# tgcsaba/GPSig

Hardware: AMD Instinct MI355X
Metric: sequence-pairs/sec for SignatureKernel.K (N,L,d,sig_level); fp64 rel-err vs ref (higher is better)
Workload: dtype f64; 1 GPU; BASELINE.json configs[1]: full N x N Gram, SignatureLinear, N=4096, L=64, d=8, num_levels=5, order=1, normalization=on, fp64, white-noise inputs

## Files before the change

gpsig_amd/csrc/ctx.hpp:

```cpp
#pragma once
#include <atomic>

#include <hip/hip_runtime.h>

#include <cstdarg>
#include <cstdio>
#include <cstdlib>
#include <cstring>
#include <string>
#include <thread>
#include <vector>

#include "../../include/gpsig_hip.h"
#include "seq_args.hpp"

struct DevBuf {
    void* p = nullptr;
    size_t cap = 0;
};

struct UploadCache {
    uint64_t hash = 0;
    void* base = nullptr;
    std::vector<size_t> offsets;
};

enum BufId {
    B_IN0, B_IN1, B_IN2,
    B_OUT0, B_OUT1, B_OUT2,
    B_REC0, B_REC1,
    B_DLEV0, B_DLEV1,
    B_FAC0, B_FAC1,
    B_TASKS, B_W, B_XT, B_ZT, B_ZS, B_ZL, B_ZN, B_TMP0, B_TMP1,
    B_LS, B_LR0, B_LR1, B_LR2, B_LR3, B_LR4, B_LR5, B_LR6, B_LR7, B_LR8,
    B_GR0, B_GR1, B_GR2, B_GR3, B_GR4, B_GR5, B_GR6, B_GR7,
    B_GR7B, B_TW0, B_TW1, B_TW2,
    B_SF0, B_SF1, B_SF2, B_SF3, B_SF4, B_SF5,
    B_SPEC,
    B_SPECD, B_LRDK,
    B_SPECW,
    B_LRF32,
    B_TQ,
    B_STASH,
    B_WD0, B_WD1, B_WD2, B_WD3, B_WD4, B_WD5, B_WD6, B_WD7, B_WD8, B_WD9, B_WD10, B_WD11, B_WD12, B_WD13, B_WD14, B_WD15,
    B_WS0, B_WS1, B_WS2, B_WS3,
    B_RG0, B_RG1, B_RG2, B_RG3, B_RG4,
    B_COUNT
};

inline thread_local std::string g_create_error;

struct TaskCache {
    int64_t key[10] = {0};
    int ntasks = 0;
    bool valid = false;
    bool match(const int64_t (&k)[10]) const {
        if (!valid) return false;
        for (int i = 0; i < 10; ++i) if (key[i] != k[i]) return false;
        return true;
    }
    void set(const int64_t (&k)[10], int n) { for (int i = 0; i < 10; ++i) key[i] = k[i]; ntasks = n; valid = true; }
};

struct TaskSlot {
    TaskCache tc;
    DevBuf buf;
    uint64_t stamp = 0;
    int64_t aux = 0;
};
constexpr size_t TASK_SLOTS = 16;

inline int64_t next_stash_generation() {
    static std::atomic<int64_t> counter{0};
    return ++counter;
}

struct gpsig_ctx {
    int device = 0;
    int num_cus = 256;
    hipStream_t stream = nullptr;
    int ptr_mode = GPSIG_PTR_HOST;
    int shard_i = 0, shard_n = 1;
    int use_glds = 1;
    int allow_exact = 1;
    int keep_reset = 1;
    int f32_pack = 2, f32_waves = 0;
    int allow_pk2 = 1;
    int max_run = 0;
    int tens_lanes = -1;
    int grad_scratch_mb = 4096;
    int matern_fast = 1;
    int grad_fused_piece = 0;
    int grad_stash_mb = 4096;
    bool stash_want = false;
    int64_t stash_desc[8] = {0, 0, 0, 0, 0, 0, 0, 0};
    int64_t stash_gen = 0;
    int grad_impl = 0;
    void* blas_handle = nullptr;
    int tvs_tile = -1;
// ... 400 lines not shown
```

gpsig_amd/csrc/launchers.hpp:

```cpp
#pragma once
#include <hip/hip_runtime.h>

#include <cstddef>
#include <cstdint>
#include <string>

struct gpsig_ctx;
struct gpsig_params;

namespace gpsig {
struct ScaleParams;
struct SeqGramArgs;
struct TvsArgs;
struct TvsLaneTArgs;
struct TvsTileArgs;
struct TvsGradTileArgs;
struct SigFeatArgs;
struct SigGramArgs;
struct SigReduceArgs;
struct SigFeatGradArgs;
struct WaveGradArgs;
struct Wave2Args;
struct WaveHoArgs;
struct FusedGradArgs;
// ... 41 lines not shown
GPSIG_SEQ_UNITS(GPSIG_SEQ_UNIT_DECL)
GPSIG_SEQ_HO_UNITS(GPSIG_SEQ_HO_UNIT_DECL)
#undef GPSIG_SEQ_UNIT_DECL
#undef GPSIG_SEQ_HO_UNIT_DECL
SeqLaunchFn seq_lookup_ptdrbf_stash(int G, int C, int D, int MMAX);
SeqLaunchFn seq_lookup_ptdmatern_stash(int kind, int G, int C, int D, int MMAX);
SeqLaunchFn seq_lookup_ho_ptdrbf_exact(int G, int C, int D, int M, int order);
SeqLaunchFn seq_lookup_ho_ptdrbf_exact_o4(int G, int C, int D, int M, int order);
SeqLaunchFn seq_lookup_ho_ptdm12_exact(int kind, int G, int C, int D, int M, int order);
SeqLaunchFn seq_lookup_ho_ptdm32_exact(int kind, int G, int C, int D, int M, int order);
SeqLaunchFn seq_lookup_ho_ptdm52_exact(int kind, int G, int C, int D, int M, int order);
bool seq_pk2_select(int rows, int d, int M, int* G, int* C, int* D);
SeqLaunchFn seq_pk2_lookup(int G, int C, int D, int M, int mode, int pack, int waves);

TvsLaunchFn tvs_lookup(int M, int TT, bool incr, bool f32);
#define GPSIG_TENS_DECL(tag) TvsLaunchFn tvs_lookup_##tag##_lo(int, int, bool); TvsLaunchFn tvs_lookup_##tag##_m6(int, int, bool); \
                             TvsLaunchFn tvs_lookup_##tag##_m7(int, int, bool); TvsLaunchFn tvs_lookup_##tag##_m8(int, int, bool);
GPSIG_TENS_DECL(f64) GPSIG_TENS_DECL(f32)
#undef GPSIG_TENS_DECL
bool tvs_lanet_plan(int M, int d, bool incr, TvsLaneTLaunchFn* fns, int* ngroups);
int tvs_tile_width(int d);
int tvs_tile_waves(int M, int D, int E, int kind);
TvsTileLaunchFn tvs_tile_lookup(int M, int NW, int D, bool incr, int kind);
TvsTileLaunchFn tvs_tile_lookup_m2(int, int, bool, int);
TvsTileLaunchFn tvs_tile_lookup_m3(int, int, bool, int);
TvsTileLaunchFn tvs_tile_lookup_m4(int, int, bool, int);
TvsTileLaunchFn tvs_tile_lookup_m5(int, int, bool, int);
TvsTileLaunchFn tvs_tile_lookup_m6(int, int, bool, int);
TvsTileLaunchFn tvs_tile_lookup_ho(int M, int NW, int D, bool incr);
TvsGradTileLaunchFn tvs_grad_tile_lookup_m1(int, int, bool);
TvsGradTileLaunchFn tvs_grad_tile_lookup_m2(int, int, bool);
TvsGradTileLaunchFn tvs_grad_tile_lookup_m3(int, int, bool);
TvsGradTileLaunchFn tvs_grad_tile_lookup_m4(int, int, bool);
TvsGradTileLaunchFn tvs_grad_tile_lookup_m5(int, int, bool);
TvsGradTileLaunchFn tvs_grad_tile_lookup_m6(int, int, bool);
TvsGradTileLaunchFn tvs_grad_tile_lookup_ho(int M, int D, bool paired, int kind);
bool tvs_grad_tile_ho_available(const gpsig_ctx* c, const gpsig_params* p, int d, int L, int increments);
int tvs_grad_tile_device(gpsig_ctx* c, const gpsig_params* p, int d, const double* Z, const double* X, const double* G, int64_t Tn, int64_t N,
                         int L, int increments, const double* fac, const double* aux, double* gZ, double* gX, double* gfac, double* gb, size_t budget, bool* done);

SigFeatLaunchFn sig_feat_lookup(int d, int M);
SigFeatLaunchFn sig_feat_pick_a(int d, int M);
SigFeatLaunchFn sig_feat_pick_b(int d, int M);
SigFeatLaunchFn sig_feat_pick_c(int d, int M);
SigFeatLaunchFn sig_feat_pick_d(int d, int M);
SigFeatLaunchFn sig_feat_pick_e(int d, int M);
SigFeatLaunchFn sig_feat_pick_f(int d, int M);
SigFeatGradLaunchFn sig_feat_grad_pick_a(int d, int M);
SigFeatGradLaunchFn sig_feat_grad_pick_b(int d, int M);
SigFeatGradLaunchFn sig_feat_grad_pick_c(int d, int M);
SigFeatGradLaunchFn sig_feat_grad_pick_d(int d, int M);
SigFeatGradLaunchFn sig_feat_grad_pick_e(int d, int M);
SigFeatGradLaunchFn sig_feat_grad_pick_f(int d, int M);
hipError_t sig_gram_launch(const SigGramArgs& G, int ntiles, hipStream_t stream, int dma, int* used_dma);
hipError_t sig_reduce_launch(const SigReduceArgs& R, hipStream_t stream);
hipError_t sig_convert_launch(const void* in, void* out, int64_t n, bool widen, hipStream_t stream);
struct SigShape { int d, M; bool cosine; int64_t F, ld; SigFeatLaunchFn ffn; };
bool sig_shape(const gpsig_params* p, int d, SigShape* s);
constexpr size_t SIG_FEAT_LDS_MAX = 150 * 1024, SIG_FEAT_GRAD_LDS_MAX = 158 * 1024;
bool sig_shape_fits(const SigShape& s, const gpsig_params* p, int L);
int sig_launch_features(gpsig_ctx* c, const SigShape& s, const gpsig_params* p, const ScaleParams& P, int order, const double* X, int64_t N, int L,
                        const double* w, int normalize, double jitter, int norm_squared, int natural_order, double* Phi, double* dlev);
int sig_features_K(gpsig_ctx* c, const gpsig_params* p, bool raw, const void* X, const void* X2, int64_t N1, int64_t N2, int L1, int L2, int return_levels,
                   void* out, bool timed, int x_squared, int64_t row_begin, int64_t row_end, int compact, bool* done, bool row_block_call = false);
bool tvs_features_plan(gpsig_ctx* c, const gpsig_params* p, bool f64, int64_t Tn, int64_t N, int L);
int tens_vs_seq_features_device(gpsig_ctx* c, const gpsig_params* p, bool f64, const void* ZT, const void* ZS, const void* X, int64_t Tn, int64_t N, int L,
                                int increments, const double* w, void* out, bool* done);
int sig_features_grad(gpsig_ctx* c, const gpsig_params* p, int d, const double* X, const double* Y, int64_t N1, int64_t N2, int L1, int L2, bool diag,
                      bool sym, const double* G, double* gX, double* gY, bool* done);

WaveLaunchFn wave_lookup_inc(int G, int C, int DP, int LQ);
WaveLaunchFn wave_lookup_ptd(int G, int C, int DP, int LQ);
WaveLaunchFn wave_lookup_ptn(int G, int C, int DP, int LQ);
Wave2LaunchFn wave2_lookup_inc(int G, int C, int DP, int LQ);
Wave2LaunchFn lam_undo_lookup_ptd_rbf(int G, int C, int DP, int LQ);
Wave2LaunchFn lam_undo_lookup_ptd_gen(int G, int C, int DP, int LQ);
Wave2LaunchFn lam_undo_lookup_ptn_rbf(int G, int C, int DP, int LQ);
Wave2LaunchFn lam_undo_lookup_ptn_gen(int G, int C, int DP, int LQ);
WaveHoLaunchFn wave_ho_lookup(int G, int C, int order, int M);
WaveHoLaunchFn wave_o1_lookup(int G, int C, int M);
WaveHoLaunchFn wave_ho_undo_lookup_g16(int C, int order, int M);
WaveHoLaunchFn wave_ho_undo_lookup_g32(int C, int order, int M);
WaveHoLaunchFn wave_ho_undo_lookup_g64(int C, int order, int M);
WaveHoLaunchFn wave_ho_levels_lookup_g16(int C, int order, int M);
WaveHoLaunchFn wave_ho_levels_lookup_g32(int C, int order, int M);
WaveHoLaunchFn wave_ho_levels_lookup_g64(int C, int order, int M);
FusedGradLaunchFn fused_grad_stash_lookup(int kind, int DP, int LQ);
FusedGradLaunchFn fused_grad_lookup_diff_g16(int kind, int DP, int LQ);
FusedGradLaunchFn fused_grad_lookup_diff_g32(int kind, int DP, int LQ);
FusedGradLaunchFn fused_grad_lookup_diff_g64(int kind, int DP, int LQ);
FusedGradLaunchFn fused_grad_lookup_nodiff_g16(int kind, int DP, int LQ);
FusedGradLaunchFn fused_grad_lookup_nodiff_g32(int kind, int DP, int LQ);
FusedGradLaunchFn fused_grad_lookup_nodiff_g64(int kind, int DP, int LQ);
struct HoSweeps { WaveHoLaunchFn fn; int G, C; size_t lds, slot; };
bool ho_sweeps_plan(const gpsig_ctx* c, const gpsig_params* p, int R1, int R2, HoSweeps* hs);
bool o1_sweeps_plan(const gpsig_ctx* c, const gpsig_params* p, int R1, int R2, HoSweeps* hs);
bool ho_levels_plan(const gpsig_ctx* c, const gpsig_params* p, int R1, int R2, HoSweeps* hs);
int ho_sweeps_launch(gpsig_ctx* c, const HoSweeps& hs, int M, int R1, int R2, const double* dM, double* lam, const double* G, int64_t gm, int64_t gi,
                     int64_t gj, int64_t N2, bool diag, int64_t pair0, int64_t npairs);
int ho_levels_launch(gpsig_ctx* c, const HoSweeps& hs, int M, int R1, int R2, const double* dM, double* out, int64_t gm, int64_t gi, int64_t gj, int64_t N2,
                     bool diag, int64_t pair0, int64_t npairs);

bool wide_tvs_available(const gpsig_ctx* c, const gpsig_params* p, int d, int64_t Tn, int64_t N, int L);
int wide_tvs_forward(gpsig_ctx* c, const gpsig_params* p, const ScaleParams& sz, int d, const double* Z, const double* Xs, int64_t Tn, int64_t N, int L,
                     int increments, const double* fx, const double* w, int sum_levels, double* out, double* aux);
int wide_tvs_backward(gpsig_ctx* c, const gpsig_params* p, int d, const double* Z, const double* X, const double* G, int64_t Tn, int64_t N, int L,
                      int increments, const double* fac, const double* aux, double* gZ, double* gX, double* gfac, double* g_base);
// ... 44 lines not shown
```

gpsig_amd/csrc/sig_feat_api.hip:

```cpp
#include "api_common.hpp"
#include "launchers.hpp"
#include "sig_feat_kernel.hpp"

namespace {

static __global__ void tens_level_features_kernel(const double* __restrict__ ZT, const double* __restrict__ ZS, int lt, int E, int d, int64_t Tn,
                                                  int M, int unit, int64_t ld, double* __restrict__ Zf) {
    const int64_t total = Tn * ld;
    for (int64_t e = blockIdx.x * int64_t(blockDim.x) + threadIdx.x; e < total; e += int64_t(gridDim.x) * blockDim.x) {
        const int64_t t = e / ld;
        int k = int(e - t * ld), m = 1, w = d, off = 0;
        while (m <= M && k >= off + w) { off += w; ++m; w *= d; }
        double v;
        if (m > M) {
            v = k == off ? 1.0 : 0.0;
        } else {
            int idx = k - off;
            const int c0 = m * (m - 1) / 2;
            v = 1.0;
            for (int j = m - 1; j >= 0; --j) {
                const int f = idx % d;
                idx /= d;
                const int c = c0 + j;
                double z = ZT[((t * d + f) * lt + c) * E + (E - 1)];
// ... 104 lines not shown
uint64_t sig_keep_key(const gpsig_params* p, bool raw, int x_squared, int64_t N1, int L1, int64_t ld) {
    const int32_t head[8] = {p->base_kernel, p->dtype, p->num_features, p->num_levels, p->order, p->difference, p->normalization, p->num_lags};
    const int64_t tail[4] = {N1, L1, (raw ? 1 : 0) + (x_squared ? 2 : 0), ld};
    uint64_t key = fnv1a(FNV1A_BASIS, head, sizeof(head));
    key = fnv1a(fnv1a(key, &p->sigma, sizeof(double)), &p->jitter, sizeof(double));
    key = fnv1a(key, p->variances, sizeof(double) * (p->num_levels + 1));
    if (p->lengthscales) key = fnv1a(key, p->lengthscales, sizeof(double) * p->num_features);
    if (p->num_lags > 0) key = fnv1a(fnv1a(key, p->lags, sizeof(double) * p->num_lags), p->gamma, sizeof(double) * (p->num_lags + 1));
    return fnv1a(key, tail, sizeof(tail));
}

int sig_gram_stage_f32(gpsig_ctx* c, const gpsig_params* p, const SigGramPlan& g, int L1, int L2, int return_levels, const void** X, const void** X2,
                       void** out) {
    void *x64, *y64 = nullptr, *o64;
    const int64_t per1 = int64_t(L1) * p->num_features, per2 = int64_t(L2) * p->num_features;
    CHK(ensure(c, B_SF3, sizeof(double) * size_t(g.N1 * per1) + 64, &x64));
    HIPCHK(c, sig_convert_launch(*X, x64, g.N1 * per1, true, c->stream));
    if (!g.sym) {
        CHK(ensure(c, B_SF4, sizeof(double) * size_t(g.N2 * per2) + 64, &y64));
        HIPCHK(c, sig_convert_launch(*X2, y64, g.N2 * per2, true, c->stream));
    }
    CHK(ensure(c, B_SF5, sizeof(double) * size_t(return_levels ? p->num_levels + 1 : 1) * size_t(g.N1) * size_t(g.sym ? g.N1 : g.N2) + 64, &o64));
    *X = x64; *X2 = g.sym ? nullptr : y64; *out = o64;
    return GPSIG_OK;
}

int sig_gram_levels(gpsig_ctx* c, const gpsig_params* p, const SigShape& s, const SigGramPlan& g, bool raw, int return_levels, int normalize,
                    const void* phi1, const void* phi2, void* part, void* out, bool timed, int compact) {
    const int M = s.M, d = s.d;
    const int64_t F = s.F, ld = s.ld, N1 = g.N1, NA = g.NA, NB = g.NB, H = g.H, row_begin = g.row_begin, Ncols = g.sym ? N1 : g.N2;
    const bool rows = g.rows;
    const int nlev = return_levels ? M + 1 : 1;
    for (int lv = 0; lv < nlev; ++lv) {
        int kb = 0, ke = int(F) + 1;
        double dval = 0.0;
        if (return_levels) {
            if (lv == 0) { kb = int(F); ke = int(F) + 1; }
            else { kb = sig_feature_count(d, lv - 1); ke = sig_feature_count(d, lv); }
            dval = raw ? 0.0 : p->sigma * p->variances[lv];
        } else {
            for (int m = 0; m <= M; ++m) dval += p->sigma * p->variances[m];
        }
        SigGramArgs G;
        memset(&G, 0, sizeof(G));
        G.A = static_cast<const double*>(phi1) + (rows ? row_begin * ld : 0);
        G.B = static_cast<const double*>(g.sym ? phi1 : phi2);
        G.NA = NA; G.NB = NB; G.lda = ld; G.ldb = ld;
        G.b_off = rows ? ((row_begin - H) % N1 + N1) % N1 : 0; G.b_mod = g.sym ? N1 : g.N2;
        G.k_begin = kb; G.k_end = ke;
        G.band = (rows && NA + H <= N1) ? H : 0;
        const int nslab = (ke - kb + SG_BK - 1) / SG_BK;
        const int ns = sig_piece_bounds(nslab, g.nsplit, return_levels ? 1 : g.graded, G.bound);
        G.nsplit = ns; G.symmetric = g.symtiles ? 1 : 0; G.ntj = g.ntj; G.part = static_cast<double*>(part);
        hipEvent_t e0 = nullptr, e1 = nullptr;
        bool on = false;
        if (timed) CHK(timing_begin(c, &e0, &e1, &on));
        int used_dma = 0;
        HIPCHK(c, sig_gram_launch(G, g.ntiles, c->stream, (c->sig_gemm_dma && !return_levels) ? 1 : 0, &used_dma));
        if (on) {
            HIPCHK(c, hipEventRecord(e1, c->stream));
            c->t_launches += 1;
            c->t_pairs += NA * NB;
            c->t_kernel = used_dma ? "sig_gram_dma_kernel" : "sig_gram_kernel";
            const double tiles_done = double(g.ntiles) - ((used_dma && g.symtiles) ? double(g.nti) * 28.0 / 64.0 : 0.0);
            c->t_flops += 2.0 * tiles_done * SG_BM * SG_BN * double(nslab) * SG_BK;
        }
        SigReduceArgs R;
        memset(&R, 0, sizeof(R));
        R.part = static_cast<const double*>(part); R.nsplit = ns; R.NA = NA; R.NB = NB;
        R.out = static_cast<double*>(out) + (return_levels ? int64_t(lv) * N1 * Ncols : 0);
        R.so_i = Ncols; R.so_j = 1;
        R.mode = rows ? 2 : (g.symtiles ? 1 : 0);
        R.diag_set = (g.sym && normalize) ? 1 : 0; R.diag_value = dval;
        R.N = N1; R.r0 = row_begin; R.c0 = G.b_off; R.compact = compact;
        HIPCHK(c, sig_reduce_launch(R, c->stream));
    }
    return GPSIG_OK;
}

}

int sig_features_K(gpsig_ctx* c, const gpsig_params* p, bool raw, const void* X, const void* X2, int64_t N1, int64_t N2, int L1, int L2,
                   int return_levels, void* out, bool timed, int x_squared, int64_t row_begin, int64_t row_end, int compact, bool* done,
                   bool row_block_call) {
    *done = false;
    const bool sym = X2 == nullptr, f32 = p->dtype == GPSIG_F32;
    const bool rows = row_end > 0 || row_block_call;
    SigShape s;
    if (!sig_gram_route(c, p, raw, sym, rows, N1, N2, L1, L2, x_squared, &s)) return GPSIG_OK;
    SigGramPlan g = sig_gram_geometry(sym, rows, N1, N2, row_begin, row_end);
    const int nslab_all = int((s.ld + SG_BK - 1) / SG_BK);
    sig_piece_counts(N1, N2, sym, nslab_all, c->sig_graded != 0, &g.nsplit, &g.graded);
    const size_t part_one = sizeof(double) * size_t(g.NA) * g.NB;
    while (g.nsplit > 1 && part_one * size_t(g.nsplit - 1 + g.graded) > (size_t(40) << 30)) { --g.nsplit; g.graded = 1; }
    const int npieces = g.nsplit - 1 + g.graded;
    const size_t feat_bytes = sizeof(double) * size_t(s.ld) * (size_t(N1) + (sym ? 0 : size_t(N2)));
    if (feat_bytes + part_one * size_t(npieces) > (size_t(96) << 30)) return GPSIG_OK;
    const SigBuf bufs[3] = {{B_SF0, sizeof(double) * size_t(s.ld) * N1 + 64}, {B_SF1, sym ? 0 : sizeof(double) * size_t(s.ld) * N2 + 64},
                            {B_SF2, part_one * size_t(npieces) + 64}};
    if (!sig_gram_headroom(c, bufs, rows)) return GPSIG_OK;
    if (rows && g.NA <= 0) { *done = true; return GPSIG_OK; }
    const double* w = nullptr;
    if (!raw) CHK(upload_weights(c, p, &w));
    ScaleParams sp;
    CHK(scale_params(c, p, !raw, &sp));
    void* dev[3] = {nullptr, nullptr, nullptr};
    for (int i = 0; i < 3; ++i)
        if (bufs[i].bytes) CHK(ensure(c, bufs[i].id, bufs[i].bytes, &dev[i]));
    void* const phi1 = dev[0];
    void* out32 = nullptr;
    const void* const X_given = X;
    if (f32) {
        out32 = out;
        CHK(sig_gram_stage_f32(c, p, g, L1, L2, return_levels, &X, &X2, &out));
    }
    const int normalize = (!raw && p->normalization) ? 1 : 0;
    const uint64_t key = sig_keep_key(p, raw, x_squared, N1, L1, s.ld);
    const bool reuse = c->sf_keep && c->sf_valid && c->sf_X == X_given && c->sf_phi == phi1 && c->sf_key == key;
    if (N1 > 0 && !reuse)
        CHK(sig_launch_features(c, s, p, sp, p->order, static_cast<const double*>(X), N1, L1, w, normalize, p->jitter, x_squared ? 1 : 0, 0,
                                static_cast<double*>(phi1), nullptr));
    c->sf_valid = c->sf_keep != 0 && N1 > 0;
    c->sf_X = X_given; c->sf_phi = phi1; c->sf_key = key;
    if (!sym && N2 > 0)
        CHK(sig_launch_features(c, s, p, sp, p->order, static_cast<const double*>(X2), N2, L2, w, normalize, p->jitter, 0, 0,
                                static_cast<double*>(dev[1]), nullptr));
    if (g.NA <= 0 || g.NB <= 0) { *done = true; return GPSIG_OK; }
    CHK(sig_gram_levels(c, p, s, g, raw, return_levels, normalize, phi1, dev[1], dev[2], out, timed, compact));
// ... 66 lines not shown
```

gpsig_amd/csrc/sig_feat_inst.hip:

```cpp
#include "launchers.hpp"
#include "sig_feat_kernel.hpp"

namespace gpsig {
SigFeatLaunchFn sig_feat_lookup(int d, int M) {
    if (d < 1 || d > 32) return nullptr;
    return d <= 4 ? sig_feat_pick_a(d, M) : d <= 8 ? sig_feat_pick_b(d, M) : d <= 12 ? sig_feat_pick_c(d, M) : d <= 16 ? sig_feat_pick_d(d, M)
         : d <= 24 ? sig_feat_pick_e(d, M) : sig_feat_pick_f(d, M);
}

hipError_t sig_gram_launch(const SigGramArgs& G, int ntiles, hipStream_t stream, int dma, int* used_dma) {
    if (used_dma) *used_dma = 0;
    const bool aligned = (G.lda % 2) == 0 && (G.ldb % 2) == 0 && (reinterpret_cast<uintptr_t>(G.A) % 16) == 0 &&
                         (reinterpret_cast<uintptr_t>(G.B) % 16) == 0;
    const int ke_pad = (G.k_end + SG_BK - 1) / SG_BK * SG_BK;
    if (dma && aligned && G.k_begin % SG_BK == 0 && ke_pad <= G.lda && ke_pad <= G.ldb) {
        hipLaunchKernelGGL(sig_gram_dma_kernel, dim3(unsigned(ntiles) * unsigned(G.nsplit)), dim3(256), 0, stream, G);
        if (used_dma) *used_dma = 1;
        return hipGetLastError();
    }
    const bool vec = (G.k_begin % 2) == 0 && (G.lda % 2) == 0 && (G.ldb % 2) == 0 && (reinterpret_cast<uintptr_t>(G.A) % 16) == 0 &&
                     (reinterpret_cast<uintptr_t>(G.B) % 16) == 0;
    if (vec) hipLaunchKernelGGL(sig_gram_kernel<true>, dim3(unsigned(ntiles) * unsigned(G.nsplit)), dim3(256), 0, stream, G);
    else hipLaunchKernelGGL(sig_gram_kernel<false>, dim3(unsigned(ntiles) * unsigned(G.nsplit)), dim3(256), 0, stream, G);
    return hipGetLastError();
}
hipError_t sig_convert_launch(const void* in, void* out, int64_t n, bool widen, hipStream_t stream) {
    if (n <= 0) return hipSuccess;
    int64_t g = (n + 255) / 256;
    if (g > 16384) g = 16384;
    if (widen) hipLaunchKernelGGL(sig_widen_kernel, dim3(unsigned(g)), dim3(256), 0, stream, static_cast<const float*>(in), static_cast<double*>(out), n);
    else hipLaunchKernelGGL(sig_narrow_kernel, dim3(unsigned(g)), dim3(256), 0, stream, static_cast<const double*>(in), static_cast<float*>(out), n);
    return hipGetLastError();
}
hipError_t sig_reduce_launch(const SigReduceArgs& R, hipStream_t stream) {
    if (R.mode == 1) {
        const int nt = int((R.NA + SG_BM - 1) / SG_BM);
        hipLaunchKernelGGL(sig_gram_reduce_sym_kernel, dim3((SG_BM / 32) * (SG_BM / 32), unsigned(nt * (nt + 1) / 2)), dim3(32, 8), 0, stream, R, nt);
        return hipGetLastError();
    }
    int64_t g = (R.NA * R.NB + 255) / 256;
    if (g > 65536) g = 65536;
    if (g < 1) g = 1;
    hipLaunchKernelGGL(sig_gram_reduce_kernel, dim3(unsigned(g)), dim3(256), 0, stream, R);
    return hipGetLastError();
}
}
```

gpsig_amd/csrc/sig_feat_kernel.hpp:

```cpp
#pragma once

#include <hip/hip_runtime.h>
#include <stdint.h>

#include <type_traits>

#include "aux_kernels.hpp"
#include "sig_pieces.hpp"

namespace gpsig {

constexpr int sig_ipow(int d, int m) {
    long long v = 1;
    for (int i = 0; i < m; ++i) { v *= d; if (v > (1ll << 30)) return 1 << 30; }
    return int(v);
}
constexpr int sig_lower_total(int d, int M) { int s = 0; for (int m = 1; m < M; ++m) s += sig_ipow(d, m); return s; }
constexpr int sig_feature_count(int d, int M) { int s = 0; for (int m = 1; m <= M; ++m) s += sig_ipow(d, m); return s; }
constexpr int SIG_MAX_TOP = 32768;
constexpr int sig_threads(int d, int M) {
    int t = 64;
    while (t < 512 && t * 64 < sig_ipow(d, M)) t *= 2;
    return t;
}
// ... 348 lines not shown
                double2* o2 = reinterpret_cast<double2*>(out + off);
#pragma unroll
                for (int q = 0; q < D; ++q)
#pragma unroll
                    for (int f = 0; f < D; f += 2) o2[(q * (D / 2) + f / 2) * T + tid] = double2{sc * top[q][f], sc * top[q][f + 1]};
            } else {
#pragma unroll
                for (int q = 0; q < D; ++q)
#pragma unroll
                    for (int f = 0; f < D; ++f) out[off + (q * D + f) * T + tid] = sc * top[q][f];
            }
            off += sig_ipow(D, M);
        }
        for (int64_t e = off + tid; e < A.ld; e += T) out[e] = e == off ? scale_of(0) : 0.0;
        if (A.dlev && tid <= M) A.dlev[n * (M + 1) + tid] = tid == 0 ? 1.0 : norms[tid];
    }
}

inline size_t sig_features_lds_bytes(int d, int M, int L) {
    (void)M;
    return sizeof(double) * ((size_t(L) + (d <= 64 ? 64 / d : 1)) * d + 64 + 64 + size_t(L) * d + size_t(L));
}

#ifdef GPSIG_KERNEL_DEFS
__global__ void sig_widen_kernel(const float* __restrict__ in, double* __restrict__ out, int64_t n) {
    for (int64_t i = blockIdx.x * int64_t(blockDim.x) + threadIdx.x; i < n; i += int64_t(gridDim.x) * blockDim.x) out[i] = double(in[i]);
}
#else
__global__ void sig_widen_kernel(const float* __restrict__ in, double* __restrict__ out, int64_t n);
#endif
#ifdef GPSIG_KERNEL_DEFS
__global__ void sig_narrow_kernel(const double* __restrict__ in, float* __restrict__ out, int64_t n) {
    for (int64_t i = blockIdx.x * int64_t(blockDim.x) + threadIdx.x; i < n; i += int64_t(gridDim.x) * blockDim.x) out[i] = float(in[i]);
}
#else
__global__ void sig_narrow_kernel(const double* __restrict__ in, float* __restrict__ out, int64_t n);
#endif

typedef double sig_f64x4 __attribute__((ext_vector_type(4)));
constexpr int SG_BM = 128, SG_BN = 128, SG_BK = 16, SG_LDK = SG_BK + 1;
constexpr int SG_MAX_PIECES = 144;

struct SigGramArgs {
    const double* A; const double* B;
    int64_t NA, NB, lda, ldb;
    int64_t b_off, b_mod;
    int k_begin, k_end;
    int nsplit;
    int bound[SG_MAX_PIECES + 1];
    int symmetric;
    int ntj;
    double* part;
    int64_t band;
};

__device__ inline void sig_tile_of(const SigGramArgs& G, int& split_out, int& bi, int& bj) {
    const int ntiles = gridDim.x / G.nsplit;
    const int split = blockIdx.x / ntiles;
    int tile;
    {
        const int j = blockIdx.x - split * ntiles, off = (split * ntiles) & 7, x = (off + j) & 7;
        int start = 0;
        for (int xp = 0; xp < x; ++xp) {
            const int j0 = (xp - off + 8) & 7;
            start += j0 < ntiles ? (ntiles - 1 - j0) / 8 + 1 : 0;
        }
        tile = start + ((j - ((x - off + 8) & 7)) >> 3);
    }
    {
        constexpr int SB = 8;
        if (G.symmetric) {
            const int d = int(int64_t(tile) * G.ntj / ntiles);
            if (int(int64_t(tile + 1) * G.ntj / ntiles) > d) {
                bi = bj = d;
                split_out = split;
                return;
            }
            tile -= d;
        }
        const int nti = G.symmetric ? G.ntj : (ntiles / G.ntj), nbi = (nti + SB - 1) / SB, nbj = (G.ntj + SB - 1) / SB;
        int Bi = 0, Bj = 0, hi = 0, wj = 0;
        bool found = false;
        for (Bi = 0; Bi < nbi && !found; ++Bi) {
            hi = nti - Bi * SB < SB ? nti - Bi * SB : SB;
            for (Bj = G.symmetric ? Bi : 0; Bj < nbj; ++Bj) {
                wj = G.ntj - Bj * SB < SB ? G.ntj - Bj * SB : SB;
                const int cnt = (G.symmetric && Bj == Bi) ? hi * (hi - 1) / 2 : hi * wj;
                if (tile < cnt) { found = true; break; }
                tile -= cnt;
            }
            if (found) break;
        }
        int li_, lj_;
        if (G.symmetric && Bj == Bi) {
            li_ = 0;
            int rowlen = hi - 1;
            while (tile >= rowlen) { tile -= rowlen; ++li_; --rowlen; }
            lj_ = li_ + 1 + tile;
        } else {
            li_ = tile / wj;
            lj_ = tile - li_ * wj;
        }
        bi = Bi * SB + li_;
        bj = Bj * SB + lj_;
    }
    split_out = split;
}

template <bool VEC>
static __global__ __launch_bounds__(256, 2) void sig_gram_kernel(const SigGramArgs G) {
    __shared__ double As[2][SG_BM * SG_LDK];
    __shared__ double Bs[2][SG_BN * SG_LDK];
    const int tid = threadIdx.x, wave = tid >> 6, lane = tid & 63;
    const int wr = wave >> 1, wc = wave & 1;
    const int li = lane & 15, lk = lane >> 4;
    int split, bi, bj;
    sig_tile_of(G, split, bi, bj);
    const int64_t tile_i = int64_t(bi) * SG_BM, tile_j = int64_t(bj) * SG_BN;
    if (G.band > 0 && (tile_j + SG_BN - 1 < tile_i || tile_j > tile_i + SG_BM - 1 + G.band)) return;
    const int s0 = G.bound[split], s1 = G.bound[split + 1];
    const int kb = G.k_begin + s0 * SG_BK, ke = (G.k_begin + s1 * SG_BK < G.k_end) ? G.k_begin + s1 * SG_BK : G.k_end;
    const int srow = tid >> 1, scol = (tid & 1) * 8;
    const int64_t ai = tile_i + srow, bjr = tile_j + srow;
    const bool aok = ai < G.NA, bok = bjr < G.NB;
    int64_t brow_i = G.b_off + (bok ? bjr : 0);
    if (brow_i >= G.b_mod) brow_i -= G.b_mod;
    const double* arow = G.A + (aok ? ai : 0) * G.lda;
    const double* brow = G.B + brow_i * G.ldb;
    double pa[8], pb[8];
    auto fetch = [&](int k0) {
        if (VEC && k0 + SG_BK <= ke) {
            const double2* a2 = reinterpret_cast<const double2*>(arow + k0 + scol);
            const double2* b2 = reinterpret_cast<const double2*>(brow + k0 + scol);
#pragma unroll
            for (int e = 0; e < 4; ++e) {
                const double2 va = a2[e], vb = b2[e];
                pa[2 * e] = va.x; pa[2 * e + 1] = va.y;
                pb[2 * e] = vb.x; pb[2 * e + 1] = vb.y;
            }
        } else {
#pragma unroll
            for (int e = 0; e < 8; ++e) {
                const int k = k0 + scol + e;
                pa[e] = (aok && k < ke) ? arow[k] : 0.0;
                pb[e] = (bok && k < ke) ? brow[k] : 0.0;
            }
        }
    };
    auto stash = [&](int buf) {
#pragma unroll
        for (int e = 0; e < 8; ++e) {
            As[buf][srow * SG_LDK + scol + e] = pa[e];
            Bs[buf][srow * SG_LDK + scol + e] = pb[e];
        }
    };
    sig_f64x4 acc[4][4];
#pragma unroll
    for (int m = 0; m < 4; ++m)
#pragma unroll
        for (int n = 0; n < 4; ++n) acc[m][n] = sig_f64x4{0.0, 0.0, 0.0, 0.0};
    if (kb < ke) {
        fetch(kb);
        stash(0);
    }
    __syncthreads();
    int buf = 0;
    for (int k0 = kb; k0 < ke; k0 += SG_BK, buf ^= 1) {
        const bool more = k0 + SG_BK < ke;
        if (more) fetch(k0 + SG_BK);
#pragma unroll
        for (int kk = 0; kk < SG_BK; kk += 4) {
            double av[4], bv[4];
#pragma unroll
            for (int m = 0; m < 4; ++m) {
                av[m] = As[buf][(wr * 64 + m * 16 + li) * SG_LDK + kk + lk];
                bv[m] = Bs[buf][(wc * 64 + m * 16 + li) * SG_LDK + kk + lk];
            }
#pragma unroll
            for (int m = 0; m < 4; ++m)
#pragma unroll
                for (int n = 0; n < 4; ++n) acc[m][n] = __builtin_amdgcn_mfma_f64_16x16x4f64(av[m], bv[n], acc[m][n], 0, 0, 0);
            if (kk == SG_BK - 8 && more) stash(buf ^ 1);
        }
        __syncthreads();
    }
    double* const P = G.part + int64_t(split) * G.NA * G.NB;
#pragma unroll
    for (int m = 0; m < 4; ++m)
#pragma unroll
        for (int n = 0; n < 4; ++n)
#pragma unroll
            for (int r = 0; r < 4; ++r) {
                const int64_t i = tile_i + wr * 64 + m * 16 + lk + 4 * r, j = tile_j + wc * 64 + n * 16 + li;
                if (i < G.NA && j < G.NB) P[i * G.NB + j] = acc[m][n][r];
            }
}


__host__ __device__ inline bool sig_gram_diag_owned(int r, int c) { return (r >> 4) <= (c >> 4); }

#ifdef GPSIG_KERNEL_DEFS
template <int W>
__device__ __forceinline__ void sig_gram_diag_tile(const SigGramArgs& G, int split, int64_t tile_i, int s0, int nsl, double* As, int lane) {
    constexpr int NF = 8 - W;
    constexpr int RB = NF - 1 - W;
    const int li = lane & 15, lk = lane >> 4;
    const double* ga[4];
#pragma unroll
    for (int q = 0; q < 4; ++q) {
        const int r = (q * 4 + W) * 8 + (lane >> 3), p = (lane & 7) ^ ((r >> 1) & 7);
        const int64_t ai = tile_i + r;
        ga[q] = G.A + (ai < G.NA ? ai : 0) * G.lda + G.k_begin + int64_t(s0) * SG_BK + 2 * p;
    }
    auto dma = [&](auto buf_c, auto ahead_c) {
        constexpr int BUF = decltype(buf_c)::value, OFF = decltype(ahead_c)::value * SG_BK * 8;
#pragma unroll
        for (int q = 0; q < 4; ++q)
            __builtin_amdgcn_global_load_lds((const __attribute__((address_space(1))) void*)ga[q],
                                             (__attribute__((address_space(3))) void*)(As + BUF * SG_BM * SG_BK + (q * 4 + W) * 8 * SG_BK - OFF / 8), 16, OFF, 0);
    };
    const int swz = (lk >> 1) ^ ((li >> 1) & 7);
    int fo[4];
#pragma unroll
    for (int kq = 0; kq < 4; ++kq) fo[kq] = (((2 * kq) ^ swz) << 1) + (lk & 1) + li * SG_BK;
    const double* const Aw = As + W * 16 * SG_BK;
    auto frag = [&](auto buf_c, int kq, double (&f)[NF]) {
        constexpr int BUF = decltype(buf_c)::value;
#pragma unroll
        for (int t = 0; t < NF; ++t) f[t] = Aw[BUF * SG_BM * SG_BK + t * 16 * SG_BK + fo[kq]];
    };
    sig_f64x4 acc_a[NF], acc_b[W + 1];
#pragma unroll
    for (int t = 0; t < NF; ++t) acc_a[t] = sig_f64x4{0.0, 0.0, 0.0, 0.0};
#pragma unroll
    for (int u = 0; u <= W; ++u) acc_b[u] = sig_f64x4{0.0, 0.0, 0.0, 0.0};
    double f[2][NF];
    using B0 = std::integral_constant<int, 0>;
    using B1 = std::integral_constant<int, 1>;
    if (nsl > 0) dma(B0{}, B0{});
    asm volatile("s_waitcnt vmcnt(0)" ::: "memory");
    __syncthreads();
    if (nsl > 0) frag(B0{}, 0, f[0]);
    auto slab = [&](auto buf_c, auto ahead_c, bool more) {
        constexpr int BUF = decltype(buf_c)::value;
        using OTHER = std::integral_constant<int, BUF ^ 1>;
        if (more) dma(OTHER{}, ahead_c);
#pragma unroll
        for (int kq = 0; kq < 4; ++kq) {
            const int cur = kq & 1, nxt = cur ^ 1;
            if (kq < 3) {
                frag(buf_c, kq + 1, f[nxt]);
            } else {
                asm volatile("s_waitcnt vmcnt(0)" ::: "memory");
                __syncthreads();
                if (more) frag(OTHER{}, 0, f[nxt]);
            }
#pragma unroll
            for (int t = 0; t < NF; ++t) acc_a[t] = __builtin_amdgcn_mfma_f64_16x16x4f64(f[cur][0], f[cur][t], acc_a[t], 0, 0, 0);
#pragma unroll
            for (int u = 0; u <= W; ++u) acc_b[u] = __builtin_amdgcn_mfma_f64_16x16x4f64(f[cur][RB], f[cur][RB + u], acc_b[u], 0, 0, 0);
        }
    };
    int s = 0;
    for (; s + 2 <= nsl; s += 2) {
        slab(B0{}, std::integral_constant<int, 1>{}, true);
        slab(B1{}, std::integral_constant<int, 2>{}, s + 2 < nsl);
#pragma unroll
        for (int q = 0; q < 4; ++q) ga[q] += 2 * SG_BK;
    }
    if (s < nsl) slab(B0{}, std::integral_constant<int, 1>{}, false);
    double* const P = G.part + int64_t(split) * G.NA * G.NB;
    auto store = [&](int sr, int sc, const sig_f64x4& a) {
#pragma unroll
        for (int r = 0; r < 4; ++r) {
            const int64_t i = tile_i + sr * 16 + lk + 4 * r, j = tile_i + sc * 16 + li;
            if (i < G.NA && j < G.NB) P[i * G.NB + j] = a[r];
        }
    };
#pragma unroll
    for (int t = 0; t < NF; ++t) store(W, W + t, acc_a[t]);
#pragma unroll
    for (int u = 0; u <= W; ++u) store(7 - W, 7 - W + u, acc_b[u]);
}

__global__ __launch_bounds__(256, 2) void sig_gram_dma_kernel(const SigGramArgs G) {
    constexpr int SG_GUARD = 8 * SG_BK;
    __shared__ __attribute__((aligned(16))) double lds_all[SG_GUARD + 2 * SG_BM * SG_BK + 2 * SG_BN * SG_BK];
    double (*const As)[SG_BM * SG_BK] = reinterpret_cast<double (*)[SG_BM * SG_BK]>(lds_all + SG_GUARD);
    double (*const Bs)[SG_BN * SG_BK] = reinterpret_cast<double (*)[SG_BN * SG_BK]>(lds_all + SG_GUARD + 2 * SG_BM * SG_BK);
    const int tid = threadIdx.x, wave = __builtin_amdgcn_readfirstlane(threadIdx.x >> 6), lane = tid & 63;
    const int wr = wave >> 1, wc = wave & 1;
    const int li = lane & 15, lk = lane >> 4;
    int split, bi, bj;
    sig_tile_of(G, split, bi, bj);
    const int64_t tile_i = int64_t(bi) * SG_BM, tile_j = int64_t(bj) * SG_BN;
    if (G.band > 0 && (tile_j + SG_BN - 1 < tile_i || tile_j > tile_i + SG_BM - 1 + G.band)) return;
    const int s0 = G.bound[split], s1 = G.bound[split + 1];
    const int nsl = s1 - s0;
    if (G.symmetric && bi == bj) {
        if (wave == 0) sig_gram_diag_tile<0>(G, split, tile_i, s0, nsl, As[0], lane);
        else if (wave == 1) sig_gram_diag_tile<1>(G, split, tile_i, s0, nsl, As[0], lane);
        else if (wave == 2) sig_gram_diag_tile<2>(G, split, tile_i, s0, nsl, As[0], lane);
        else sig_gram_diag_tile<3>(G, split, tile_i, s0, nsl, As[0], lane);
        return;
    }
    const double* ga[4];
    const double* gb[4];
#pragma unroll
    for (int q = 0; q < 4; ++q) {
        const int r = (q * 4 + wave) * 8 + (lane >> 3), p = (lane & 7) ^ ((r >> 1) & 7);
        const int64_t ai = tile_i + r, bjr = tile_j + r;
        int64_t brow_i = G.b_off + (bjr < G.NB ? bjr : 0);
        if (brow_i >= G.b_mod) brow_i -= G.b_mod;
        ga[q] = G.A + (ai < G.NA ? ai : 0) * G.lda + G.k_begin + int64_t(s0) * SG_BK + 2 * p;
        gb[q] = G.B + brow_i * G.ldb + G.k_begin + int64_t(s0) * SG_BK + 2 * p;
    }
    auto dma = [&](auto buf_c, auto ahead_c) {
        constexpr int BUF = decltype(buf_c)::value, OFF = decltype(ahead_c)::value * SG_BK * 8;
#pragma unroll
        for (int q = 0; q < 4; ++q) {
            __builtin_amdgcn_global_load_lds((const __attribute__((address_space(1))) void*)ga[q],
                                             (__attribute__((address_space(3))) void*)(&As[BUF][(q * 4 + wave) * 8 * SG_BK] - OFF / 8), 16, OFF, 0);
            __builtin_amdgcn_global_load_lds((const __attribute__((address_space(1))) void*)gb[q],
                                             (__attribute__((address_space(3))) void*)(&Bs[BUF][(q * 4 + wave) * 8 * SG_BK] - OFF / 8), 16, OFF, 0);
        }
    };
    auto advance = [&](int slabs) {
#pragma unroll
        for (int q = 0; q < 4; ++q) { ga[q] += slabs * SG_BK; gb[q] += slabs * SG_BK; }
    };
    const int swz = (lk >> 1) ^ ((li >> 1) & 7);
    int fo[4];
#pragma unroll
    for (int kq = 0; kq < 4; ++kq) fo[kq] = (((2 * kq) ^ swz) << 1) + (lk & 1) + li * SG_BK;
    const double* const Aw = &As[0][wr * 64 * SG_BK];
    const double* const Bw = &Bs[0][wc * 64 * SG_BK];
    auto frag = [&](auto buf_c, int kq, double (&av)[4], double (&bv)[4]) {
        constexpr int BUF = decltype(buf_c)::value;
#pragma unroll
        for (int m = 0; m < 4; ++m) {
            av[m] = Aw[BUF * SG_BM * SG_BK + m * 16 * SG_BK + fo[kq]];
            bv[m] = Bw[BUF * SG_BN * SG_BK + m * 16 * SG_BK + fo[kq]];
        }
    };
    sig_f64x4 acc[4][4];
#pragma unroll
    for (int m = 0; m < 4; ++m)
#pragma unroll
        for (int n = 0; n < 4; ++n) acc[m][n] = sig_f64x4{0.0, 0.0, 0.0, 0.0};
    double fa[2][4], fb[2][4];
    using B0 = std::integral_constant<int, 0>;
    using B1 = std::integral_constant<int, 1>;
    if (nsl > 0) dma(B0{}, B0{});
    asm volatile("s_waitcnt vmcnt(0)" ::: "memory");
    __syncthreads();
    if (nsl > 0) frag(B0{}, 0, fa[0], fb[0]);
    auto slab = [&](auto buf_c, auto ahead_c, bool more) {
        constexpr int BUF = decltype(buf_c)::value;
        using OTHER = std::integral_constant<int, BUF ^ 1>;
        if (more) dma(OTHER{}, ahead_c);
#pragma unroll
        for (int kq = 0; kq < 4; ++kq) {
            const int cur = kq & 1, nxt = cur ^ 1;
            if (kq < 3) {
                frag(buf_c, kq + 1, fa[nxt], fb[nxt]);
            } else {
                asm volatile("s_waitcnt vmcnt(0)" ::: "memory");
                __syncthreads();
                if (more) frag(OTHER{}, 0, fa[nxt], fb[nxt]);
            }
#pragma unroll
            for (int m = 0; m < 4; ++m)
#pragma unroll
                for (int n = 0; n < 4; ++n) acc[m][n] = __builtin_amdgcn_mfma_f64_16x16x4f64(fa[cur][m], fb[cur][n], acc[m][n], 0, 0, 0);
        }
    };
    int s = 0;
    for (; s + 8 <= nsl; s += 8) {
        slab(B0{}, std::integral_constant<int, 1>{}, true);
        slab(B1{}, std::integral_constant<int, 2>{}, true);
        slab(B0{}, std::integral_constant<int, 3>{}, true);
        slab(B1{}, std::integral_constant<int, 4>{}, true);
        slab(B0{}, std::integral_constant<int, 5>{}, true);
        slab(B1{}, std::integral_constant<int, 6>{}, true);
        slab(B0{}, std::integral_constant<int, 7>{}, true);
        slab(B1{}, std::integral_constant<int, 8>{}, s + 8 < nsl);
        advance(8);
    }
    for (; s + 2 <= nsl; s += 2) {
        slab(B0{}, std::integral_constant<int, 1>{}, true);
        slab(B1{}, std::integral_constant<int, 2>{}, s + 2 < nsl);
        advance(2);
    }
    if (s < nsl) slab(B0{}, std::integral_constant<int, 1>{}, false);
    double* const P = G.part + int64_t(split) * G.NA * G.NB;
#pragma unroll
    for (int m = 0; m < 4; ++m)
#pragma unroll
        for (int n = 0; n < 4; ++n)
#pragma unroll
            for (int r = 0; r < 4; ++r) {
                const int64_t i = tile_i + wr * 64 + m * 16 + lk + 4 * r, j = tile_j + wc * 64 + n * 16 + li;
                if (i < G.NA && j < G.NB) P[i * G.NB + j] = acc[m][n][r];
            }
}
#else
__global__ __launch_bounds__(256, 2) void sig_gram_dma_kernel(const SigGramArgs G);
#endif

struct SigReduceArgs {
    const double* part; int nsplit; int64_t NA, NB;
    double* out; int64_t so_i, so_j;
    int mode, diag_set; double diag_value;
    int64_t N, r0, c0;
    int compact;
};
#ifdef GPSIG_KERNEL_DEFS
__global__ void sig_gram_reduce_sym_kernel(const SigReduceArgs R, int nt) {
    __shared__ double tile[32][33];
    int t = blockIdx.y, bi = 0, rowlen = nt;
    while (t >= rowlen) { t -= rowlen; ++bi; --rowlen; }
    const int bj = bi + t;
    constexpr int SB = SG_BM / 32;
    const int sbi = blockIdx.x / SB, sbj = blockIdx.x - sbi * SB;
    const int64_t i0 = int64_t(bi) * SG_BM + sbi * 32, j0 = int64_t(bj) * SG_BN + sbj * 32;
    const int64_t stride = R.NA * R.NB;
    if (bi == bj && sbi > sbj) return;
    const bool dblock = bi == bj && sbi == sbj;
    for (int r = threadIdx.y; r < 32; r += 8) {
        const int64_t i = i0 + r, j = j0 + threadIdx.x;
        double s = 0.0;
        if (i < R.NA && j < R.NB && (!dblock || sig_gram_diag_owned(r, threadIdx.x))) {
            for (int k = 0; k < R.nsplit; ++k) s += R.part[int64_t(k) * stride + i * R.NB + j];
            if (i == j && R.diag_set) s = R.diag_value;
            R.out[i * R.so_i + j * R.so_j] = s;
        }
        tile[r][threadIdx.x] = s;
    }
    __syncthreads();
    for (int r = threadIdx.y; r < 32; r += 8) {
        const int64_t j = j0 + r, i = i0 + threadIdx.x;
        if (i < R.NA && j < R.NB && (!dblock || !sig_gram_diag_owned(r, threadIdx.x))) R.out[j * R.so_i + i * R.so_j] = tile[threadIdx.x][r];
    }
}
#else
__global__ void sig_gram_reduce_sym_kernel(const SigReduceArgs R, int nt);
#endif

#ifdef GPSIG_KERNEL_DEFS
__global__ void sig_gram_reduce_kernel(const SigReduceArgs R) {
    const int64_t total = R.NA * R.NB, stride = R.NA * R.NB;
    for (int64_t e = blockIdx.x * int64_t(blockDim.x) + threadIdx.x; e < total; e += int64_t(gridDim.x) * blockDim.x) {
        const int64_t i = e / R.NB, j = e - i * R.NB;
        int64_t src = e;
        if (R.mode == 1 && (i / SG_BM) > (j / SG_BN)) src = j * R.NB + i;
        double s = 0.0;
        if (R.mode == 2) {
// ... 25 lines not shown
```

Measured before the change: 1.783 billion sequence-pairs/s.

## Fold split-K reduction into gram DMA kernel via last-arriver atomic ticket

For the symmetric full-Gram DMA path, each split-K block now takes an atomic ticket per tile after writing its partials. The last block to arrive sums all partial slabs, applies the normalization diagonal, and writes both the tile and its mirrored transpose into the output. This removes the separate reduce kernel launch and its extra pass over the partial buffer. In exchange it adds a counter buffer with a memset, fences and atomics, and a serialized tail of reduce work in the final block of each tile.

```diff
diff --git a/gpsig_amd/csrc/ctx.hpp b/gpsig_amd/csrc/ctx.hpp
--- a/gpsig_amd/csrc/ctx.hpp
+++ b/gpsig_amd/csrc/ctx.hpp
@@ -45,6 +45,7 @@
     B_WD0, B_WD1, B_WD2, B_WD3, B_WD4, B_WD5, B_WD6, B_WD7, B_WD8, B_WD9, B_WD10, B_WD11, B_WD12, B_WD13, B_WD14, B_WD15,
     B_WS0, B_WS1, B_WS2, B_WS3,
     B_RG0, B_RG1, B_RG2, B_RG3, B_RG4,
+    B_SFC,
     B_COUNT
 };
 
diff --git a/gpsig_amd/csrc/launchers.hpp b/gpsig_amd/csrc/launchers.hpp
--- a/gpsig_amd/csrc/launchers.hpp
+++ b/gpsig_amd/csrc/launchers.hpp
@@ -117,7 +117,7 @@
 SigFeatGradLaunchFn sig_feat_grad_pick_d(int d, int M);
 SigFeatGradLaunchFn sig_feat_grad_pick_e(int d, int M);
 SigFeatGradLaunchFn sig_feat_grad_pick_f(int d, int M);
-hipError_t sig_gram_launch(const SigGramArgs& G, int ntiles, hipStream_t stream, int dma, int* used_dma);
+hipError_t sig_gram_launch(const SigGramArgs& G, int ntiles, hipStream_t stream, int dma, int* used_dma, int* folded);
 hipError_t sig_reduce_launch(const SigReduceArgs& R, hipStream_t stream);
 hipError_t sig_convert_launch(const void* in, void* out, int64_t n, bool widen, hipStream_t stream);
 struct SigShape { int d, M; bool cosine; int64_t F, ld; SigFeatLaunchFn ffn; };
diff --git a/gpsig_amd/csrc/sig_feat_api.hip b/gpsig_amd/csrc/sig_feat_api.hip
--- a/gpsig_amd/csrc/sig_feat_api.hip
+++ b/gpsig_amd/csrc/sig_feat_api.hip
@@ -180,11 +180,27 @@
         const int nslab = (ke - kb + SG_BK - 1) / SG_BK;
         const int ns = sig_piece_bounds(nslab, g.nsplit, return_levels ? 1 : g.graded, G.bound);
         G.nsplit = ns; G.symmetric = g.symtiles ? 1 : 0; G.ntj = g.ntj; G.part = static_cast<double*>(part);
+        SigReduceArgs R;
+        memset(&R, 0, sizeof(R));
+        R.part = static_cast<const double*>(part); R.nsplit = ns; R.NA = NA; R.NB = NB;
+        R.out = static_cast<double*>(out) + (return_levels ? int64_t(lv) * N1 * Ncols : 0);
+        R.so_i = Ncols; R.so_j = 1;
+        R.mode = rows ? 2 : (g.symtiles ? 1 : 0);
+        R.diag_set = (g.sym && normalize) ? 1 : 0; R.diag_value = dval;
+        R.N = N1; R.r0 = row_begin; R.c0 = G.b_off; R.compact = compact;
+        if (R.mode == 1 && !return_levels && c->sig_gemm_dma) {
+            void* cnt = nullptr;
+            const size_t cnt_bytes = (sizeof(int) * size_t(g.ntiles) + 15) / 16 * 16;
+            CHK(ensure(c, B_SFC, cnt_bytes, &cnt));
+            if (ns > 1 && !c->capturing) HIPCHK(c, hipMemsetAsync(cnt, 0, cnt_bytes, c->stream));
+            G.fold = 1; G.cnt = static_cast<int*>(cnt);
+            G.out = R.out; G.so_i = R.so_i; G.so_j = R.so_j; G.diag_set = R.diag_set; G.diag_value = R.diag_value;
+        }
         hipEvent_t e0 = nullptr, e1 = nullptr;
         bool on = false;
         if (timed) CHK(timing_begin(c, &e0, &e1, &on));
-        int used_dma = 0;
-        HIPCHK(c, sig_gram_launch(G, g.ntiles, c->stream, (c->sig_gemm_dma && !return_levels) ? 1 : 0, &used_dma));
+        int used_dma = 0, folded = 0;
+        HIPCHK(c, sig_gram_launch(G, g.ntiles, c->stream, (c->sig_gemm_dma && !return_levels) ? 1 : 0, &used_dma, &folded));
         if (on) {
             HIPCHK(c, hipEventRecord(e1, c->stream));
             c->t_launches += 1;
@@ -193,15 +209,7 @@
             const double tiles_done = double(g.ntiles) - ((used_dma && g.symtiles) ? double(g.nti) * 28.0 / 64.0 : 0.0);
             c->t_flops += 2.0 * tiles_done * SG_BM * SG_BN * double(nslab) * SG_BK;
         }
-        SigReduceArgs R;
-        memset(&R, 0, sizeof(R));
-        R.part = static_cast<const double*>(part); R.nsplit = ns; R.NA = NA; R.NB = NB;
-        R.out = static_cast<double*>(out) + (return_levels ? int64_t(lv) * N1 * Ncols : 0);
-        R.so_i = Ncols; R.so_j = 1;
-        R.mode = rows ? 2 : (g.symtiles ? 1 : 0);
-        R.diag_set = (g.sym && normalize) ? 1 : 0; R.diag_value = dval;
-        R.N = N1; R.r0 = row_begin; R.c0 = G.b_off; R.compact = compact;
-        HIPCHK(c, sig_reduce_launch(R, c->stream));
+        if (!folded) HIPCHK(c, sig_reduce_launch(R, c->stream));
     }
     return GPSIG_OK;
 }
diff --git a/gpsig_amd/csrc/sig_feat_inst.hip b/gpsig_amd/csrc/sig_feat_inst.hip
--- a/gpsig_amd/csrc/sig_feat_inst.hip
+++ b/gpsig_amd/csrc/sig_feat_inst.hip
@@ -8,16 +8,21 @@
          : d <= 24 ? sig_feat_pick_e(d, M) : sig_feat_pick_f(d, M);
 }
 
-hipError_t sig_gram_launch(const SigGramArgs& G, int ntiles, hipStream_t stream, int dma, int* used_dma) {
+hipError_t sig_gram_launch(const SigGramArgs& G_in, int ntiles, hipStream_t stream, int dma, int* used_dma, int* folded) {
     if (used_dma) *used_dma = 0;
+    if (folded) *folded = 0;
+    SigGramArgs G = G_in;
     const bool aligned = (G.lda % 2) == 0 && (G.ldb % 2) == 0 && (reinterpret_cast<uintptr_t>(G.A) % 16) == 0 &&
                          (reinterpret_cast<uintptr_t>(G.B) % 16) == 0;
     const int ke_pad = (G.k_end + SG_BK - 1) / SG_BK * SG_BK;
     if (dma && aligned && G.k_begin % SG_BK == 0 && ke_pad <= G.lda && ke_pad <= G.ldb) {
+        G.groups = G.fold ? SG_FOLD_GROUPS : 1;
         hipLaunchKernelGGL(sig_gram_dma_kernel, dim3(unsigned(ntiles) * unsigned(G.nsplit)), dim3(256), 0, stream, G);
         if (used_dma) *used_dma = 1;
+        if (folded) *folded = G.fold ? 1 : 0;
         return hipGetLastError();
     }
+    G.fold = 0; G.groups = 1;
     const bool vec = (G.k_begin % 2) == 0 && (G.lda % 2) == 0 && (G.ldb % 2) == 0 && (reinterpret_cast<uintptr_t>(G.A) % 16) == 0 &&
                      (reinterpret_cast<uintptr_t>(G.B) % 16) == 0;
     if (vec) hipLaunchKernelGGL(sig_gram_kernel<true>, dim3(unsigned(ntiles) * unsigned(G.nsplit)), dim3(256), 0, stream, G);
diff --git a/gpsig_amd/csrc/sig_feat_kernel.hpp b/gpsig_amd/csrc/sig_feat_kernel.hpp
--- a/gpsig_amd/csrc/sig_feat_kernel.hpp
+++ b/gpsig_amd/csrc/sig_feat_kernel.hpp
@@ -424,21 +424,38 @@
     int ntj;
     double* part;
     int64_t band;
+    int fold;
+    int groups;
+    int* cnt;
+    double* out; int64_t so_i, so_j;
+    int diag_set; double diag_value;
 };
 
-__device__ inline void sig_tile_of(const SigGramArgs& G, int& split_out, int& bi, int& bj) {
+constexpr int SG_FOLD_GROUPS = 1;
+
+__device__ inline void sig_tile_of(const SigGramArgs& G, int& split_out, int& bi, int& bj, int& tile_out) {
     const int ntiles = gridDim.x / G.nsplit;
-    const int split = blockIdx.x / ntiles;
+    int t0 = 0, t1 = ntiles;
+    if (G.groups > 1) {
+        int g = 0;
+        for (int gg = 1; gg < G.groups; ++gg)
+            if (int(int64_t(ntiles) * gg / G.groups) * G.nsplit <= int(blockIdx.x)) g = gg;
+        t0 = int(int64_t(ntiles) * g / G.groups);
+        t1 = int(int64_t(ntiles) * (g + 1) / G.groups);
+    }
+    const int ng = t1 - t0, base = t0 * G.nsplit;
+    const int split = (int(blockIdx.x) - base) / ng;
     int tile;
     {
-        const int j = blockIdx.x - split * ntiles, off = (split * ntiles) & 7, x = (off + j) & 7;
+        const int j = int(blockIdx.x) - base - split * ng, off = (base + split * ng) & 7, x = (off + j) & 7;
         int start = 0;
         for (int xp = 0; xp < x; ++xp) {
             const int j0 = (xp - off + 8) & 7;
-            start += j0 < ntiles ? (ntiles - 1 - j0) / 8 + 1 : 0;
-        }
-        tile = start + ((j - ((x - off + 8) & 7)) >> 3);
-    }
+            start += j0 < ng ? (ng - 1 - j0) / 8 + 1 : 0;
+        }
+        tile = t0 + start + ((j - ((x - off + 8) & 7)) >> 3);
+    }
+    tile_out = tile;
     {
         constexpr int SB = 8;
         if (G.symmetric) {
@@ -486,8 +503,9 @@
     const int tid = threadIdx.x, wave = tid >> 6, lane = tid & 63;
     const int wr = wave >> 1, wc = wave & 1;
     const int li = lane & 15, lk = lane >> 4;
-    int split, bi, bj;
-    sig_tile_of(G, split, bi, bj);
+    int split, bi, bj, tile;
+    sig_tile_of(G, split, bi, bj, tile);
+    (void)tile;
     const int64_t tile_i = int64_t(bi) * SG_BM, tile_j = int64_t(bj) * SG_BN;
     if (G.band > 0 && (tile_j + SG_BN - 1 < tile_i || tile_j > tile_i + SG_BM - 1 + G.band)) return;
     const int s0 = G.bound[split], s1 = G.bound[split + 1];
@@ -572,6 +590,84 @@
 __host__ __device__ inline bool sig_gram_diag_owned(int r, int c) { return (r >> 4) <= (c >> 4); }
 
 #ifdef GPSIG_KERNEL_DEFS
+constexpr int SG_FOLD_ROWS = 32, SG_FOLD_LD = SG_BN + 1;
+__device__ __forceinline__ void sig_gram_fold(const SigGramArgs& G, int tile, int bi, int bj, double* lds, int tid) {
+    static_assert(SG_BN == 128 && SG_BM % SG_FOLD_ROWS == 0, "thread = (column, row parity) of a 128-column strip");
+    asm volatile("s_waitcnt vmcnt(0)" ::: "memory");
+    __syncthreads();
+    if (G.nsplit > 1) {
+        int* const flag = reinterpret_cast<int*>(lds);
+        if (tid == 0) {
+            __builtin_amdgcn_fence(__ATOMIC_RELEASE, "agent");
+            asm volatile("s_waitcnt vmcnt(0)" ::: "memory");
+            const int ticket = __hip_atomic_fetch_add((__attribute__((address_space(1))) int*)(G.cnt + tile), 1, __ATOMIC_RELAXED, __HIP_MEMORY_SCOPE_AGENT);
+            const int last = ticket == G.nsplit - 1 ? 1 : 0;
+            if (last) {
+                __hip_atomic_store((__attribute__((address_space(1))) int*)(G.cnt + tile), 0, __ATOMIC_RELAXED, __HIP_MEMORY_SCOPE_AGENT);
+                __builtin_amdgcn_fence(__ATOMIC_ACQUIRE, "agent");
+                asm volatile("s_waitcnt vmcnt(0)" ::: "memory");
+            }
+            *flag = last;
+        }
+        __syncthreads();
+        if (*flag == 0) return;
+    }
+    double* const S = lds + 16;
+    const int c = tid & (SG_BN - 1), rh = tid >> 7;
+    const bool diag = bi == bj;
+    const int64_t tile_i = int64_t(bi) * SG_BM, tile_j = int64_t(bj) * SG_BN, j = tile_j + c;
+    const int64_t stride = G.NA * G.NB;
+    const char* const P0 = reinterpret_cast<const char*>(G.part + tile_i * G.NB + tile_j);
+    constexpr int NQ = SG_FOLD_ROWS / 2;
+    auto owned = [&](int r) { return tile_i + r < G.NA && j < G.NB && (!diag || sig_gram_diag_owned(r, c)); };
+    for (int r0 = 0; r0 < SG_BM && tile_i + r0 < G.NA; r0 += SG_FOLD_ROWS) {
+        unsigned off[NQ];
+        double s[NQ], v0[NQ], v1[NQ];
+#pragma unroll
+        for (int q = 0; q < NQ; ++q) {
+            const int r = r0 + rh + 2 * q;
+            off[q] = owned(r) ? unsigned(r * G.NB + c) * unsigned(sizeof(double)) : 0u;
+            s[q] = 0.0;
+        }
+        auto load = [&](double (&v)[NQ], int k) {
+            const auto rsrc = __builtin_amdgcn_make_buffer_rsrc(const_cast<char*>(P0 + int64_t(k) * stride * int64_t(sizeof(double))), 0, -1, 0x00020000);
+#pragma unroll
+            for (int q = 0; q < NQ; ++q) v[q] = __builtin_bit_cast(double, __builtin_amdgcn_raw_buffer_load_b64(rsrc, int(off[q]), 0, 0));
+        };
+        auto add = [&](const double (&v)[NQ]) {
+#pragma unroll
+            for (int q = 0; q < NQ; ++q) s[q] += v[q];
+        };
+        int k = 0;
+        load(v0, 0);
+        for (; k + 1 < G.nsplit; k += 2) {
+            load(v1, k + 1);
+            add(v0);
+            if (k + 2 < G.nsplit) load(v0, k + 2);
+            add(v1);
+        }
+        if (k < G.nsplit) add(v0);
+#pragma unroll
+        for (int q = 0; q < NQ; ++q) {
+            const int r = r0 + rh + 2 * q;
+            const int64_t i = tile_i + r;
+            if (owned(r)) {
+                if (i == j && G.diag_set) s[q] = G.diag_value;
+                G.out[i * G.so_i + j * G.so_j] = s[q];
+            }
+            S[(r - r0) * SG_FOLD_LD + c] = s[q];
+        }
+        __syncthreads();
+        const int il = tid & (SG_FOLD_ROWS - 1);
+        const int64_t i = tile_i + r0 + il;
+        for (int jl = tid / SG_FOLD_ROWS; jl < SG_BN; jl += 256 / SG_FOLD_ROWS) {
+            const int64_t jj = tile_j + jl;
+            if (i < G.NA && jj < G.NB && (!diag || !sig_gram_diag_owned(jl, r0 + il))) G.out[jj * G.so_i + i * G.so_j] = S[il * SG_FOLD_LD + jl];
+        }
+        __syncthreads();
+    }
+}
+
 template <int W>
 __device__ __forceinline__ void sig_gram_diag_tile(const SigGramArgs& G, int split, int64_t tile_i, int s0, int nsl, double* As, int lane) {
     constexpr int NF = 8 - W;
@@ -658,13 +754,14 @@
 __global__ __launch_bounds__(256, 2) void sig_gram_dma_kernel(const SigGramArgs G) {
     constexpr int SG_GUARD = 8 * SG_BK;
     __shared__ __attribute__((aligned(16))) double lds_all[SG_GUARD + 2 * SG_BM * SG_BK + 2 * SG_BN * SG_BK];
+    static_assert(sizeof(lds_all) >= sizeof(double) * (16 + SG_FOLD_ROWS * SG_FOLD_LD), "sig_gram_fold's strip lives in this array after the loop");
     double (*const As)[SG_BM * SG_BK] = reinterpret_cast<double (*)[SG_BM * SG_BK]>(lds_all + SG_GUARD);
     double (*const Bs)[SG_BN * SG_BK] = reinterpret_cast<double (*)[SG_BN * SG_BK]>(lds_all + SG_GUARD + 2 * SG_BM * SG_BK);
     const int tid = threadIdx.x, wave = __builtin_amdgcn_readfirstlane(threadIdx.x >> 6), lane = tid & 63;
     const int wr = wave >> 1, wc = wave & 1;
     const int li = lane & 15, lk = lane >> 4;
-    int split, bi, bj;
-    sig_tile_of(G, split, bi, bj);
+    int split, bi, bj, tile;
+    sig_tile_of(G, split, bi, bj, tile);
     const int64_t tile_i = int64_t(bi) * SG_BM, tile_j = int64_t(bj) * SG_BN;
     if (G.band > 0 && (tile_j + SG_BN - 1 < tile_i || tile_j > tile_i + SG_BM - 1 + G.band)) return;
     const int s0 = G.bound[split], s1 = G.bound[split + 1];
@@ -674,6 +771,7 @@
         else if (wave == 1) sig_gram_diag_tile<1>(G, split, tile_i, s0, nsl, As[0], lane);
         else if (wave == 2) sig_gram_diag_tile<2>(G, split, tile_i, s0, nsl, As[0], lane);
         else sig_gram_diag_tile<3>(G, split, tile_i, s0, nsl, As[0], lane);
+        if (G.fold) sig_gram_fold(G, tile, bi, bj, lds_all, tid);
         return;
     }
     const double* ga[4];
@@ -775,6 +873,7 @@
                 const int64_t i = tile_i + wr * 64 + m * 16 + lk + 4 * r, j = tile_j + wc * 64 + n * 16 + li;
                 if (i < G.NA && j < G.NB) P[i * G.NB + j] = acc[m][n][r];
             }
+    if (G.fold) sig_gram_fold(G, tile, bi, bj, lds_all, tid);
 }
 #else
 __global__ __launch_bounds__(256, 2) void sig_gram_dma_kernel(const SigGramArgs G);
```

New measurement: 1.804 billion sequence-pairs/s, median of 6. +1.2%, better.
